# sinamalakouti/CDDMSL

Measured on AMD Instinct MI355X. Metric: images/sec (train step) VOC+Clipart RN50-C4, higher is better.
Workload: dtype bf16

## Files before the change

cddmsl_amd/csrc/roi_align.hip:

```cpp
#include "common.h"

namespace {

template <typename T> struct Vec;
template <> struct Vec<__bf16> {
  static constexpr int ES = 2, VEC = 8;
  __device__ static __forceinline__ void unpack(const u32x4& v, float* f) {
#pragma unroll
    for (int j = 0; j < 4; ++j) { f[2 * j] = bf2f(v[j] & 0xffff); f[2 * j + 1] = bf2f(v[j] >> 16); }
  }
  __device__ static __forceinline__ u32x4 pack(const float* f) {
    u32x4 v;
#pragma unroll
    for (int j = 0; j < 4; ++j) v[j] = pack2bf(f[2 * j], f[2 * j + 1]);
    return v;
  }
};
template <> struct Vec<float> {
  static constexpr int ES = 4, VEC = 4;
  __device__ static __forceinline__ void unpack(const u32x4& v, float* f) {
    const f32x4 x = __builtin_bit_cast(f32x4, v);
    f[0] = x[0]; f[1] = x[1]; f[2] = x[2]; f[3] = x[3];
  }
  __device__ static __forceinline__ u32x4 pack(const float* f) {
// ... 77 lines not shown
    const int i = i0 + rr, j = j0 + cc;
    const long bin = ((long)k * ph + i) * pw + j;
    float acc[8] = {0, 0, 0, 0, 0, 0, 0, 0};
    if (g.b >= 0 && g.b < N) {
      for (int iy = 0; iy < g.gh; ++iy) {
        int yl, yh; float wyl, wyh;
        if (tabled) {
          yl = s_lo[0][rr * g.gh + iy];
          if (yl < 0) continue;
          yh = s_hi[0][rr * g.gh + iy]; wyl = s_wl[0][rr * g.gh + iy]; wyh = s_wh[0][rr * g.gh + iy];
        } else {
          float yy = g.y0 + (float)i * g.bh + ((float)iy + 0.5f) * g.bh / (float)g.gh;
          if (!axis_tap(yy, H, yl, yh, wyl, wyh)) continue;
        }
        for (int ix = 0; ix < g.gw; ++ix) {
          int xl, xh; float wxl, wxh;
          if (tabled) {
            const int sx = j * g.gw + ix;
            xl = s_lo[1][sx];
            if (xl < 0) continue;
            xh = s_hi[1][sx]; wxl = s_wl[1][sx]; wxh = s_wh[1][sx];
          } else {
            float xx = g.x0 + (float)j * g.bw + ((float)ix + 0.5f) * g.bw / (float)g.gw;
            if (!axis_tap(xx, W, xl, xh, wxl, wxh)) continue;
          }
          float v1[8], v2[8], v3[8], v4[8];
          Vec<T>::unpack(xb[((long)yl * W + xl) * cch + c], v1);
          Vec<T>::unpack(xb[((long)yl * W + xh) * cch + c], v2);
          Vec<T>::unpack(xb[((long)yh * W + xl) * cch + c], v3);
          Vec<T>::unpack(xb[((long)yh * W + xh) * cch + c], v4);
          float w1 = wyl * wxl, w2 = wyl * wxh, w3 = wyh * wxl, w4 = wyh * wxh;
#pragma unroll
          for (int q = 0; q < VEC; ++q) {
            if (sizeof(T) == 2) {
              float tq = w1 * v1[q];
              tq = __builtin_fmaf(w2, v2[q], tq);
              tq = __builtin_fmaf(w3, v3[q], tq);
              tq = __builtin_fmaf(w4, v4[q], tq);
              acc[q] += tq;
            } else {
              acc[q] += w1 * v1[q] + w2 * v2[q] + w3 * v3[q] + w4 * v4[q];
            }
          }
        }
      }
    }
    if (pow2) {
#pragma unroll
      for (int q = 0; q < VEC; ++q) acc[q] *= inv_count;
    } else {
#pragma unroll
      for (int q = 0; q < VEC; ++q) acc[q] /= count;
    }
    if (esc) {
#pragma unroll
      for (int q = 0; q < VEC; ++q) {
        const float sq = esc[c * VEC + q], bq = ebi[c * VEC + q];
        acc[q] = sizeof(T) == 2 ? __builtin_fmaf(acc[q], sq, bq) : acc[q] * sq + bq;
        if (relu) acc[q] = fmaxf(acc[q], 0.f);
      }
    }
    outp[rr][cc] = Vec<T>::pack(acc);
    if (y) ((u32x4*)y)[bin * cch + c] = outp[rr][cc];
    if (sizeof(T) == 2 && y8) {
      float f8[8];
#pragma unroll
      for (int q = 0; q < 8; ++q) { am8 = absmax_bits(am8, acc[q]); f8[q] = __builtin_amdgcn_fmed3f(acc[q] * q8s, -448.f, 448.f); }
      int w0 = __builtin_amdgcn_cvt_pk_fp8_f32(f8[0], f8[1], 0, false), w1 = __builtin_amdgcn_cvt_pk_fp8_f32(f8[4], f8[5], 0, false);
      w0 = __builtin_amdgcn_cvt_pk_fp8_f32(f8[2], f8[3], w0, true); w1 = __builtin_amdgcn_cvt_pk_fp8_f32(f8[6], f8[7], w1, true);
      const u32x2 o8 = {(unsigned)w0, (unsigned)w1};
      ((u32x2*)y8)[bin * cch + c] = o8;
    }
    }
    if (RP == 2) {
      float a0[8], a1[8], a2[8], a3[8], o[8];
      Vec<T>::unpack(outp[0][0], a0); Vec<T>::unpack(outp[0][RP - 1], a1);
      Vec<T>::unpack(outp[RP - 1][0], a2); Vec<T>::unpack(outp[RP - 1][RP - 1], a3);
#pragma unroll
      for (int q = 0; q < VEC; ++q) o[q] = ((a0[q] + a1[q]) + (a2[q] + a3[q])) * 0.25f;
      ((u32x4*)yp)[(((long)k * (ph / 2) + i0 / 2) * (pw / 2) + j0 / 2) * cch + c] = Vec<T>::pack(o);
    }
  }
  }
  if (sizeof(T) == 2 && y8 && amax8) {
    __shared__ unsigned sm8[4];
    am8 = wave_max_u(am8);
    if ((threadIdx.x & 63) == 0) sm8[threadIdx.x >> 6] = am8;
    __syncthreads();
    if (threadIdx.x == 0) {
      unsigned m = sm8[0];
      for (int wv = 1; wv < (int)(blockDim.x >> 6); ++wv) m = sm8[wv] > m ? sm8[wv] : m;
      atomicMax(amax8 + (blockIdx.x & 63), m);
    }
  }
}

constexpr int ROW_MAXY = 32;
template <int RP>
__global__ __launch_bounds__(256) void k_roi_align_fwd_rows(const char* x, const float* rois, char* y, int N, int H, int W, int cch, int ph, int pw,
                                                            float scale, int sampling_ratio, int aligned, const float* esc, const float* ebi, int relu) {
  const int nrb = ph / RP;
  const int i0 = (blockIdx.x % nrb) * RP, k = blockIdx.x / nrb;
  const RoiGeom g = roi_geom(rois + 5 * (long)k, scale, ph, pw, sampling_ratio, aligned);
  __shared__ int s_xl[ROI_MAXS], s_py[ROW_MAXY], s_n[2];
  __shared__ float s_xwl[ROI_MAXS], s_xwh[ROI_MAXS], s_wy[ROW_MAXY];
  __shared__ int s_ylo[ROW_MAXY], s_yhi[ROW_MAXY];
  __shared__ float s_ywl[ROW_MAXY], s_ywh[ROW_MAXY];
  const int ny = RP * g.gh, nx = pw * g.gw;
  const int opw = pw / RP;
  const int c = threadIdx.x;
  const bool inb = g.b >= 0 && g.b < N;
  if (nx > ROI_MAXS || 2 * ny > ROW_MAXY || g.bw < 0.f) {
    if (c >= cch) return;
    const u32x4* xb = (const u32x4*)x + (long)(inb ? g.b : 0) * H * W * cch + c;
    const float inv = 1.0f / ((float)max(g.gh * g.gw, 1) * (float)(RP * RP));
    for (int jo = 0; jo < opw; ++jo) {
      float acc[8] = {0, 0, 0, 0, 0, 0, 0, 0};
      for (int rr = 0; rr < RP && inb; ++rr)
        for (int cc = 0; cc < RP; ++cc)
          for (int iy = 0; iy < g.gh; ++iy) {
            int yl, yh; float wyl, wyh;
            const float yy = g.y0 + (float)(i0 + rr) * g.bh + ((float)iy + 0.5f) * g.bh / (float)g.gh;
            if (!axis_tap(yy, H, yl, yh, wyl, wyh)) continue;
            for (int ix = 0; ix < g.gw; ++ix) {
              int xl, xh; float wxl, wxh;
              const float xx = g.x0 + (float)(jo * RP + cc) * g.bw + ((float)ix + 0.5f) * g.bw / (float)g.gw;
              if (!axis_tap(xx, W, xl, xh, wxl, wxh)) continue;
              float v1[8], v2[8], v3[8], v4[8];
              Vec<__bf16>::unpack(xb[((long)yl * W + xl) * cch], v1); Vec<__bf16>::unpack(xb[((long)yl * W + xh) * cch], v2);
              Vec<__bf16>::unpack(xb[((long)yh * W + xl) * cch], v3); Vec<__bf16>::unpack(xb[((long)yh * W + xh) * cch], v4);
#pragma unroll
              for (int q = 0; q < 8; ++q) acc[q] += wyl * (wxl * v1[q] + wxh * v2[q]) + wyh * (wxl * v3[q] + wxh * v4[q]);
            }
          }
      float o[8];
#pragma unroll
      for (int q = 0; q < 8; ++q) {
        o[q] = acc[q] * inv;
        if (esc) { o[q] = __builtin_fmaf(o[q], esc[c * 8 + q], ebi[c * 8 + q]); if (relu) o[q] = fmaxf(o[q], 0.f); }
      }
      ((u32x4*)y)[(((long)k * nrb + i0 / RP) * opw + jo) * cch + c] = Vec<__bf16>::pack(o);
    }
    return;
  }
  for (int s = threadIdx.x; s < ny + nx; s += blockDim.x) {
    int lo = -1, hi = -1; float wl = 0.f, wh = 0.f;
    if (s < ny) {
      const int rr = s / g.gh, iy = s - rr * g.gh;
      const float yy = g.y0 + (float)(i0 + rr) * g.bh + ((float)iy + 0.5f) * g.bh / (float)g.gh;
      if (!axis_tap(yy, H, lo, hi, wl, wh)) lo = -1;
      s_ylo[s] = lo; s_yhi[s] = hi; s_ywl[s] = wl; s_ywh[s] = wh;
    } else {
      const int sx = s - ny, j = sx / g.gw, ix = sx - j * g.gw;
      const float xx = g.x0 + (float)j * g.bw + ((float)ix + 0.5f) * g.bw / (float)g.gw;
      if (!axis_tap(xx, W, lo, hi, wl, wh)) lo = -1;
      s_xl[sx] = lo; s_xwl[sx] = wl; s_xwh[sx] = wh;
    }
  }
  __syncthreads();
  if (threadIdx.x == 0) {
    int n = 0;
    for (int s = 0; s < ny; ++s) {
      if (s_ylo[s] < 0) continue;
      const int r2[2] = {s_ylo[s], s_yhi[s]};
      const float w2[2] = {s_ywl[s], s_ywh[s]};
      for (int e = 0; e < 2; ++e) {
        int f = -1;
        for (int q = 0; q < n; ++q) if (s_py[q] == r2[e]) f = q;
        if (f < 0) { f = n++; s_py[f] = r2[e]; s_wy[f] = 0.f; }
        s_wy[f] += w2[e];
      }
    }
    int first = -1;
    for (int s = 0; s < nx && first < 0; ++s) if (s_xl[s] >= 0) first = s_xl[s];
    s_n[0] = n; s_n[1] = first;
  }
  __syncthreads();
  const int lane = threadIdx.x & 63;
  int xlr[ROI_MAXS / 64], xwlr[ROI_MAXS / 64], xwhr[ROI_MAXS / 64];
#pragma unroll
  for (int q = 0; q < ROI_MAXS / 64; ++q) {
    const int idx = q * 64 + lane;
    const bool in = idx < nx;
    xlr[q] = in ? s_xl[idx] : -1;
    xwlr[q] = in ? __builtin_bit_cast(int, s_xwl[idx]) : 0;
    xwhr[q] = in ? __builtin_bit_cast(int, s_xwh[idx]) : 0;
  }
  if (c >= cch) return;
  const int nrow = __builtin_amdgcn_readfirstlane(s_n[0]);
  const int first = __builtin_amdgcn_readfirstlane(s_n[1]);
  const float inv = 1.0f / ((float)max(g.gh * g.gw, 1) * (float)(RP * RP));
  float sq[8], bq[8];
#pragma unroll
  for (int q = 0; q < 8; ++q) { sq[q] = esc ? esc[c * 8 + q] : 1.f; bq[q] = ebi ? ebi[c * 8 + q] : 0.f; }
  const u32x4* xb = (const u32x4*)x + (long)(inb ? g.b : 0) * H * W * cch + c;
  auto rload = [&](int px, float* R) {
#pragma unroll
    for (int q = 0; q < 8; ++q) R[q] = 0.f;
    for (int e = 0; e < nrow; ++e) {
      const int py = __builtin_amdgcn_readfirstlane(s_py[e]);
      const float wy = __builtin_bit_cast(float, __builtin_amdgcn_readfirstlane(__builtin_bit_cast(int, s_wy[e])));
      float v[8];
      Vec<__bf16>::unpack(xb[((long)py * W + px) * cch], v);
#pragma unroll
      for (int q = 0; q < 8; ++q) R[q] = __builtin_fmaf(wy, v[q], R[q]);
    }
  };
  float R0[8], R1[8], acc[8];
#pragma unroll
  for (int q = 0; q < 8; ++q) { R0[q] = R1[q] = acc[q] = 0.f; }
  int cur = first;
  const bool any = inb && nrow > 0 && first >= 0;
  constexpr int PF = 4;
  const bool ahead = nrow <= PF;
  int pyr[PF]; float wyr[PF];
#pragma unroll
  for (int e = 0; e < PF; ++e) {
    pyr[e] = __builtin_amdgcn_readfirstlane(s_py[e < nrow ? e : 0]);
    wyr[e] = e < nrow ? __builtin_bit_cast(float, __builtin_amdgcn_readfirstlane(__builtin_bit_cast(int, s_wy[e]))) : 0.f;
  }
  u32x4 raw[PF];
  auto issue = [&](int px) {
#pragma unroll
    for (int e = 0; e < PF; ++e) if (e < nrow) raw[e] = xb[((long)pyr[e] * W + px) * cch];
  };
  auto finish = [&](float* R) {
#pragma unroll
    for (int q = 0; q < 8; ++q) R[q] = 0.f;
#pragma unroll
    for (int e = 0; e < PF; ++e) if (e < nrow) {
      float v[8];
      Vec<__bf16>::unpack(raw[e], v);
#pragma unroll
      for (int q = 0; q < 8; ++q) R[q] = __builtin_fmaf(wyr[e], v[q], R[q]);
    }
  };
  if (any) {
    rload(cur, R0); rload(min(cur + 1, W - 1), R1);
    if (ahead) issue(min(cur + 2, W - 1));
  }
  const int spo = RP * g.gw;
  u32x4* yo = (u32x4*)y + ((long)k * nrb + i0 / RP) * opw * cch + c;
  if (nx == 0) {
    float o[8];
#pragma unroll
    for (int q = 0; q < 8; ++q) { o[q] = 0.f; if (esc) { o[q] = bq[q]; if (relu) o[q] = fmaxf(o[q], 0.f); } }
    for (int jo = 0; jo < opw; ++jo) yo[(long)jo * cch] = Vec<__bf16>::pack(o);
    return;
  }
  int left = spo, j = 0;
#pragma unroll
  for (int q = 0; q < ROI_MAXS / 64; ++q) {
  const int lim = min(64, nx - q * 64);
  for (int l = 0; l < lim; ++l) {
    const int xl = __builtin_amdgcn_readlane(xlr[q], l);
    if (any && xl >= 0) {
      while (cur < xl) {
        ++cur;
#pragma unroll
        for (int q = 0; q < 8; ++q) R0[q] = R1[q];
        if (ahead) { finish(R1); issue(min(cur + 2, W - 1)); }
        else rload(min(cur + 1, W - 1), R1);
      }
      const float wl = __builtin_bit_cast(float, __builtin_amdgcn_readlane(xwlr[q], l));
      const float wh = __builtin_bit_cast(float, __builtin_amdgcn_readlane(xwhr[q], l));
#pragma unroll
      for (int q = 0; q < 8; ++q) acc[q] = __builtin_fmaf(wl, R0[q], __builtin_fmaf(wh, R1[q], acc[q]));
    }
    if (--left == 0) {
      float o[8];
#pragma unroll
      for (int q = 0; q < 8; ++q) {
        o[q] = acc[q] * inv;
        if (esc) { o[q] = __builtin_fmaf(o[q], sq[q], bq[q]); if (relu) o[q] = fmaxf(o[q], 0.f); }
        acc[q] = 0.f;
      }
      __builtin_nontemporal_store(Vec<__bf16>::pack(o), &yo[(long)j * cch]);
      ++j; left = spo;
    }
  }
  }
}

__global__ void k_roi_tables(const float* rois, float* ay, float* ax, int* fp, int K, int H, int W, int ph, int pw,
                             float scale, int sampling_ratio, int aligned, int fold) {
  int k = blockIdx.x;
  RoiGeom g = roi_geom(rois + 5 * (long)k, scale, ph * fold, pw * fold, sampling_ratio, aligned);
  float* ayk = ay + (long)k * H * ph;
  float* axk = ax + (long)k * W * pw;
  for (int i = threadIdx.x; i < H * ph; i += blockDim.x) ayk[i] = 0.f;
  for (int i = threadIdx.x; i < W * pw; i += blockDim.x) axk[i] = 0.f;
  __shared__ int lim[4];
  if (threadIdx.x == 0) { lim[0] = H; lim[1] = -1; lim[2] = W; lim[3] = -1; }
  __syncthreads();
  const float fw = 1.0f / (float)fold;
  if (threadIdx.x < ph) {
    int lo_min = H, hi_max = -1;
    for (int i = threadIdx.x * fold; i < (threadIdx.x + 1) * fold; ++i)
    for (int iy = 0; iy < g.gh; ++iy) {
      float yy = g.y0 + (float)i * g.bh + ((float)iy + 0.5f) * g.bh / (float)g.gh;
      int yl, yh; float wl, wh;
      if (!axis_tap(yy, H, yl, yh, wl, wh)) continue;
      ayk[yl * ph + threadIdx.x] += fw * (wl / (float)g.gh);
      ayk[yh * ph + threadIdx.x] += fw * (wh / (float)g.gh);
      lo_min = min(lo_min, yl); hi_max = max(hi_max, yh);
    }
    atomicMin(&lim[0], lo_min); atomicMax(&lim[1], hi_max);
  } else if (threadIdx.x >= 64 && threadIdx.x < 64 + pw) {
    const int jc = threadIdx.x - 64;
    int lo_min = W, hi_max = -1;
    for (int j = jc * fold; j < (jc + 1) * fold; ++j)
    for (int ix = 0; ix < g.gw; ++ix) {
      float xx = g.x0 + (float)j * g.bw + ((float)ix + 0.5f) * g.bw / (float)g.gw;
      int xl, xh; float wl, wh;
      if (!axis_tap(xx, W, xl, xh, wl, wh)) continue;
      axk[xl * pw + jc] += fw * (wl / (float)g.gw);
      axk[xh * pw + jc] += fw * (wh / (float)g.gw);
      lo_min = min(lo_min, xl); hi_max = max(hi_max, xh);
    }
    atomicMin(&lim[2], lo_min); atomicMax(&lim[3], hi_max);
  }
  __syncthreads();
  if (threadIdx.x == 0) {
    bool ok = g.b >= 0;
    fp[4 * k] = ok ? lim[0] : 1; fp[4 * k + 1] = ok ? lim[1] : 0; fp[4 * k + 2] = lim[2]; fp[4 * k + 3] = lim[3];
  }
}

// ... 47 lines not shown
      for (int a = 0; a < TS; ++a) wyi[a] = __builtin_bit_cast(float, __builtin_amdgcn_readlane(__builtin_bit_cast(int, wyv[a]), i));
      unsigned long long xm = xm0;
      while (xm) {
        const int j = __builtin_ctzll(xm);
        xm &= xm - 1;
        float wxj[TS];
#pragma unroll
        for (int a = 0; a < TS; ++a) wxj[a] = __builtin_bit_cast(float, __builtin_amdgcn_readlane(__builtin_bit_cast(int, wxv[a]), j));
        const u32x4* src = (const u32x4*)dy + (((long)k * ph + i) * pw + j) * cch;
        float v[NC][8];
#pragma unroll
        for (int u = 0; u < NC; ++u) {
          const int c = threadIdx.x + u * blockDim.x;
          if (c < cch) Vec<T>::unpack(src[c], v[u]);
        }
#pragma unroll
        for (int a = 0; a < TS; ++a)
#pragma unroll
          for (int b = 0; b < TS; ++b) {
            const float w = wyi[a] * wxj[b];
            if (w == 0.f) continue;
#pragma unroll
            for (int u = 0; u < NC; ++u)
#pragma unroll
              for (int q = 0; q < VEC; ++q) acc[u][a * TS + b][q] += w * v[u][q];
          }
      }
    }
  }
  }
#pragma unroll
  for (int u = 0; u < NC; ++u) {
    const int c = threadIdx.x + u * blockDim.x;
    if (c < cch) {
#pragma unroll
      for (int a = 0; a < TS; ++a)
#pragma unroll
        for (int b = 0; b < TS; ++b)
          if (py0 + a < H && px0 + b < W) ((u32x4*)dx)[(((long)n * H + py0 + a) * W + px0 + b) * cch + c] = Vec<T>::pack(acc[u][a * TS + b]);
    }
  }
}

}

static int roi_align_forward_impl(const void* x, const float* rois, void* y, void* y_pooled, int* dbg_grid, const float* esc,
                                  const float* ebi, int relu, int N, int C, int H, int W, int K, int ph, int pw, float spatial_scale,
                                  int sampling_ratio, int aligned, int dtype, void* stream, void* y8 = nullptr, const float* q8 = nullptr,
                                  float* amax8 = nullptr) {
  int es = dtype == 0 ? 2 : 4;
  if ((dtype != 0 && dtype != 1) || (C * es) % 16 || H <= 0 || W <= 0 || ph <= 0 || pw <= 0 || K < 0 || N < 0)
    return CDDMSL_ERR_ARG;
  if ((esc == nullptr) != (ebi == nullptr)) return CDDMSL_ERR_ARG;
  if (K == 0) return CDDMSL_OK;
  if (!y && !y_pooled) return CDDMSL_ERR_ARG;
  if (y8 && (dtype != 0 || !y)) return CDDMSL_ERR_ARG;
  int cch = C * es / 16;
  if (y_pooled && ((ph & 1) || (pw & 1))) return CDDMSL_ERR_ARG;
  long grid = (long)K * (y_pooled ? ph / 2 : ph);
  if (grid > 0x7fffffffL) return CDDMSL_ERR_ARG;
  int threads = cch >= 256 ? 256 : ((cch + 63) / 64) * 64;
  hipStream_t st = (hipStream_t)stream;
  const char* rows_env = getenv("CDDMSL_ROI_ROWS");
  const bool rows_off = rows_env && rows_env[0] == '0';
  if (dtype == 0 && !y8 && !dbg_grid && ((y != nullptr) != (y_pooled != nullptr)) && cch <= 256 && !rows_off) {
    if (y) k_roi_align_fwd_rows<1><<<dim3((unsigned)((long)K * ph)), dim3(threads), 0, st>>>((const char*)x, rois, (char*)y, N, H, W, cch, ph, pw, spatial_scale, sampling_ratio, aligned, esc, ebi, relu);
    else k_roi_align_fwd_rows<2><<<dim3((unsigned)((long)K * (ph / 2))), dim3(threads), 0, st>>>((const char*)x, rois, (char*)y_pooled, N, H, W, cch, ph, pw, spatial_scale, sampling_ratio, aligned, esc, ebi, relu);
    return launch_status();
  }
#define CDDMSL_RAF(TT, RPP) k_roi_align_fwd<TT, RPP><<<dim3((unsigned)grid), dim3(threads), 0, st>>>((const char*)x, rois, (char*)y, (char*)y_pooled, dbg_grid, N, H, W, cch, ph, pw, spatial_scale, sampling_ratio, aligned, esc, ebi, relu, (char*)y8, q8, (unsigned*)amax8)
  if (dtype == 0) { if (y_pooled) CDDMSL_RAF(__bf16, 2); else CDDMSL_RAF(__bf16, 1); }
  else { if (y_pooled) CDDMSL_RAF(float, 2); else CDDMSL_RAF(float, 1); }
#undef CDDMSL_RAF
  return launch_status();
}

extern "C" int cddmsl_roi_align_forward(const void* x, const float* rois, void* y, void* y_pooled, int* dbg_grid, int N, int C,
                                        int H, int W, int K, int ph, int pw, float spatial_scale, int sampling_ratio,
                                        int aligned, int dtype, void* stream) {
  if (!y && K > 0) return CDDMSL_ERR_ARG;
  return roi_align_forward_impl(x, rois, y, y_pooled, dbg_grid, nullptr, nullptr, 0, N, C, H, W, K, ph, pw, spatial_scale,
                                sampling_ratio, aligned, dtype, stream);
}

extern "C" int cddmsl_roi_align_forward_affine(const void* x, const float* rois, void* y, void* y_pooled, const float* scale,
                                               const float* bias, int relu, int N, int C, int H, int W, int K, int ph, int pw,
                                               float spatial_scale, int sampling_ratio, int aligned, int dtype, void* y8,
                                               const float* q8, float* amax8, void* stream) {
  return roi_align_forward_impl(x, rois, y, y_pooled, nullptr, scale, bias, relu, N, C, H, W, K, ph, pw, spatial_scale,
                                sampling_ratio, aligned, dtype, stream, y8, q8, amax8);
}

static int roi_align_backward_impl(const void* dy, const float* rois, const int* roi_start, void* dx, float* ws_ay,
                                   float* ws_ax, int* ws_fp, int N, int C, int H, int W, int K, int ph, int pw,
                                   float spatial_scale, int sampling_ratio, int aligned, int dtype, int fold, void* stream) {
  int es = dtype == 0 ? 2 : 4;
  if ((dtype != 0 && dtype != 1) || (C * es) % 16 || H <= 0 || W <= 0 || ph <= 0 || pw <= 0 || K < 0 || N < 0)
    return CDDMSL_ERR_ARG;
  if (ph > MAXP || pw > MAXP || ph > 64 || pw > 64) return CDDMSL_ERR_ARG;
  int cch = C * es / 16;
  if (cch > 1024) return CDDMSL_ERR_ARG;
  hipStream_t st = (hipStream_t)stream;
  if (N == 0) return CDDMSL_OK;
  if (K > 0) k_roi_tables<<<dim3((unsigned)K), dim3(128), 0, st>>>(rois, ws_ay, ws_ax, ws_fp, K, H, W, ph, pw, spatial_scale, sampling_ratio, aligned, fold);
  int threads = cch >= 256 ? 256 : ((cch + 63) / 64) * 64;
  const int ncpt = (cch + threads - 1) / threads;
  const int ts = 2;
  long grid = (long)N * ((H + ts - 1) / ts) * ((W + ts - 1) / ts);
  if (grid > 0x7fffffffL) return CDDMSL_ERR_ARG;
#define CDDMSL_RAB(TT, NCC, TSS) k_roi_align_bwd<TT, NCC, TSS><<<dim3((unsigned)grid), dim3(threads), 0, st>>>((const char*)dy, ws_ay, ws_ax, ws_fp, roi_start, (char*)dx, H, W, cch, ph, pw)
  if (dtype == 0) { if (ncpt <= 1) CDDMSL_RAB(__bf16, 1, 2); else if (ncpt == 2) CDDMSL_RAB(__bf16, 2, 2); else CDDMSL_RAB(__bf16, 4, 2); }
  else { if (ncpt <= 1) CDDMSL_RAB(float, 1, 2); else if (ncpt == 2) CDDMSL_RAB(float, 2, 2); else CDDMSL_RAB(float, 4, 2); }
#undef CDDMSL_RAB
  return launch_status();
}

extern "C" int cddmsl_roi_align_backward(const void* dy, const float* rois, const int* roi_start, void* dx, float* ws_ay,
                                         float* ws_ax, int* ws_fp, int N, int C, int H, int W, int K, int ph, int pw,
                                         float spatial_scale, int sampling_ratio, int aligned, int dtype, void* stream) {
  return roi_align_backward_impl(dy, rois, roi_start, dx, ws_ay, ws_ax, ws_fp, N, C, H, W, K, ph, pw, spatial_scale,
// ... 112 lines not shown
```

cddmsl_amd/hip.py:

```python
import ctypes
import os
from ctypes import c_float, c_int, c_long, c_void_p

import torch

from ._lib import check, lib, ptr, require_cuda, stream_ptr

DT = {torch.bfloat16: 0, torch.float32: 1}

_sigs_done = False


def _L():
    global _sigs_done
    L = lib()
    if not _sigs_done:
        vp, ci, cf = c_void_p, c_int, c_float
        L.cddmsl_last_kernel.argtypes = []
        L.cddmsl_plan_only.argtypes = [ci]
        L.cddmsl_conv_fwd.argtypes = [vp] * 7 + [ci] * 16 + [vp]
        L.cddmsl_bottleneck64_ok.argtypes = [ci] * 4
        L.cddmsl_bottleneck64_fwd.argtypes = [vp] * 17 + [ci] * 4 + [vp]
        L.cddmsl_conv_wgrad.argtypes = [vp] * 4 + [ci] * 12 + [vp]
        L.cddmsl_set_workspace.argtypes = [vp, c_long]
# ... 649 lines not shown
    return dx


@_timed("colsum")
def colsum(x2d, period=1, out=None):
    require_cuda(x2d, out)
    rows, cols = x2d.shape
    assert x2d.is_contiguous()
    if out is None:
        out = torch.zeros((period, cols) if period > 1 else (cols,), device=x2d.device, dtype=torch.float32)
    check(_L().cddmsl_colsum(ptr(x2d), ptr(out), rows, cols, period, _dt(x2d), stream_ptr()), "cddmsl_colsum")
    return out


def same_layout(a, b):
    return a.shape == b.shape and all(sa == sb for sa, sb, n in zip(a.stride(), b.stride(), a.shape) if n > 1)


@_timed("sgd_clip_step")
def sgd_clip_step(params, grads, moms, norm_ws, lr, momentum, wd, clip, first_step):
    n = len(params)
    if n == 0:
        return
    require_cuda(*params, *grads, *moms)
    for p, g, m in zip(params, grads, moms):
        assert p.dtype == g.dtype == m.dtype == torch.float32
        assert same_layout(p, g) and same_layout(p, m), "param/grad/momentum must share a memory layout"
    P = (c_void_p * n)(*[p.data_ptr() for p in params])
    G = (c_void_p * n)(*[g.data_ptr() for g in grads])
    M = (c_void_p * n)(*[m.data_ptr() for m in moms])
    S = (c_long * n)(*[p.numel() for p in params])
    check(_L().cddmsl_sgd_clip_step(P, G, M, S, n, ptr(norm_ws), lr, momentum, wd, clip, int(first_step), stream_ptr()),
          "cddmsl_sgd_clip_step")


@_timed("roi_align_forward")
def roi_align_forward(x, rois, ph, pw, spatial_scale, sampling_ratio, aligned, dbg_grid=None, with_pooled=False, extra_rows=0):
    require_cuda(x, rois)
    assert rois.dim() == 2 and rois.size(1) == 5 and rois.dtype == torch.float32 and rois.is_contiguous()
    N, H, W, C = x.shape
    K = rois.shape[0]
    y = torch.empty((K + extra_rows, ph, pw, C), device=x.device, dtype=x.dtype)
    yp = torch.empty((K + extra_rows, ph // 2, pw // 2, C), device=x.device, dtype=x.dtype) if with_pooled else None
    check(_L().cddmsl_roi_align_forward(ptr(x), ptr(rois), ptr(y), ptr(yp), ptr(dbg_grid), N, C, H, W, K, ph, pw, spatial_scale,
                                         sampling_ratio, int(aligned), _dt(x), stream_ptr()), "cddmsl_roi_align_forward")
    return (y, yp) if with_pooled else y


@_timed("roi_align_forward")
def roi_align_forward_affine(x, rois, ph, pw, spatial_scale, sampling_ratio, aligned, scale=None, bias=None, relu=False,
                             pooled_only=False, extra_rows=0, emit8=None):
    require_cuda(x, rois)
    assert rois.dim() == 2 and rois.size(1) == 5 and rois.dtype == torch.float32 and rois.is_contiguous()
    assert (scale is None) == (bias is None) and not (pooled_only and scale is not None)
    N, H, W, C = x.shape
    K = rois.shape[0]
    if pooled_only:
        y, yp = None, torch.empty((K + extra_rows, ph // 2, pw // 2, C), device=x.device, dtype=x.dtype)
    else:
        y, yp = torch.empty((K + extra_rows, ph, pw, C), device=x.device, dtype=x.dtype), None
        assert scale is None or (scale.dtype == torch.float32 and scale.numel() == C and bias.numel() == C and scale.is_contiguous() and bias.is_contiguous())
    y8 = None
    if emit8 is not None:
        assert not pooled_only and x.dtype == torch.bfloat16
        y8 = torch.empty(y.shape, device=x.device, dtype=torch.uint8)
    check(_L().cddmsl_roi_align_forward_affine(ptr(x), ptr(rois), ptr(y), ptr(yp), ptr(scale), ptr(bias), int(relu), N, C, H, W, K,
                                                ph, pw, spatial_scale, sampling_ratio, int(aligned), _dt(x), ptr(y8),
                                                ptr(emit8[0]) if emit8 else c_void_p(0), ptr(emit8[1]) if emit8 else c_void_p(0), stream_ptr()),
          "cddmsl_roi_align_forward_affine")
    if y8 is not None:
        y._fp8 = (y8, emit8[0].data_ptr())
    return yp if pooled_only else y


@_timed("roi_align_backward")
def roi_align_backward(dy, rois, roi_start, in_shape, spatial_scale, sampling_ratio, aligned, pooled=False):
    require_cuda(dy, rois, roi_start)
    N, H, W, C = in_shape
    K, ph, pw, _ = dy.shape
    assert roi_start.dtype == torch.int32 and roi_start.numel() == N + 1 and dy.is_contiguous()
    dx = torch.empty(in_shape, device=dy.device, dtype=dy.dtype)
    ay = workspace("roi_ay", max(K, 1) * H * ph * 4, dy.device)
    ax = workspace("roi_ax", max(K, 1) * W * pw * 4, dy.device)
    fp = workspace("roi_fp", max(K, 1) * 16, dy.device)
    fn = _L().cddmsl_roi_align_backward_pooled if pooled else _L().cddmsl_roi_align_backward
    check(fn(ptr(dy), ptr(rois), ptr(roi_start), ptr(dx), ptr(ay), ptr(ax), ptr(fp), N, C, H, W, K,
             ph, pw, spatial_scale, sampling_ratio, int(aligned), _dt(dy), stream_ptr()), "cddmsl_roi_align_backward")
    return dx


def roi_align_nchw(input, rois, output_size, spatial_scale, sampling_ratio, aligned):
    require_cuda(input, rois)
    assert rois.dim() == 2 and rois.size(1) == 5 and rois.dtype == torch.float32 and rois.is_contiguous() and input.is_contiguous()
    N, C, H, W = input.shape
    ph, pw = (output_size, output_size) if isinstance(output_size, int) else output_size
    K = rois.shape[0]
    out = torch.zeros((K, C, ph, pw), device=input.device, dtype=input.dtype)
    nbytes = ctypes.c_size_t(0)
    args = (N, C, H, W, K, ph, pw, spatial_scale, sampling_ratio, int(aligned), _dt(input))
    check(_L().cddmsl_roi_align_nchw_anyorder(ptr(input), ptr(rois), ptr(out), *args, None, ctypes.byref(nbytes), stream_ptr()), "cddmsl_roi_align_nchw_anyorder(size)")
    ws = workspace("roi_nchw", max(nbytes.value, 1), input.device)
    check(_L().cddmsl_roi_align_nchw_anyorder(ptr(input), ptr(rois), ptr(out), *args, ptr(ws), ctypes.byref(nbytes), stream_ptr()), "cddmsl_roi_align_nchw_anyorder")
    return out


def roi_align_backward_nchw(grad, rois, input_shape, spatial_scale, sampling_ratio, aligned):
    require_cuda(grad, rois)
    assert rois.dtype == torch.float32 and rois.is_contiguous() and grad.is_contiguous()
    N, C, H, W = input_shape
    K, _, ph, pw = grad.shape
    dx = torch.zeros(tuple(input_shape), device=grad.device, dtype=grad.dtype)
    nbytes = ctypes.c_size_t(0)
    args = (N, C, H, W, K, ph, pw, spatial_scale, sampling_ratio, int(aligned), _dt(grad))
    check(_L().cddmsl_roi_align_backward_nchw_anyorder(ptr(grad), ptr(rois), ptr(dx), *args, None, ctypes.byref(nbytes), stream_ptr()), "cddmsl_roi_align_backward_nchw_anyorder(size)")
# ... 586 lines not shown
```

cddmsl_amd/layers.py:

```python
import os
import weakref

import torch

from . import hip

_STEP = [0]


def bump_weight_version():
    _STEP[0] += 1


_LOAD_GEN = [0]


def note_weights_loaded(*_):
    _LOAD_GEN[0] += 1
    _STEP[0] += 1


def load_generation():
    return _LOAD_GEN[0]

# ... 550 lines not shown


def _fused_stage_forward(x, blocks):
    T = x.dtype
    wf = lambda pw: pw.get(T, need_dgrad=False)[0]
    o1 = conv_fwd_auto(x, blocks[0].pw[0], blocks[0].bn[0][0], blocks[0].bn[0][1], False, relu=True)
    cur = x
    for bi, bp in enumerate(blocks):
        nxt = blocks[bi + 1] if bi + 1 < len(blocks) else None
        kw = dict(x0=cur, wd=wf(bp.pw[3]), bnd=bp.bn[3]) if bp.pw[3] is not None else dict(residual=cur)
        if nxt is not None:
            kw.update(w1n=wf(nxt.pw[0]), bn1n=nxt.bn[0])
        cur, o1 = hip.bottleneck64_fwd(o1, wf(bp.pw[1]), bp.bn[1], wf(bp.pw[2]), bp.bn[2], **kw)
    return cur


def res_stage(x, blocks, frozen, out_grad_premasked=False, out_spec=None):
    px0 = getattr(x, "_pooled2", None)
    if frozen or not torch.is_grad_enabled():
        if _fused_stage_ok(x, blocks, out_spec):
            return _fused_stage_forward(x, blocks)
        cur = x
        for bi, bp in enumerate(blocks):
            cur, _ = _block_forward(cur, bp, False, px0 if bi == 0 else None, blocks[bi + 1].pw[0] if bi + 1 < len(blocks) else None,
                                    out_spec if bi + 1 == len(blocks) else None)
        return cur
    return ResStageFn.apply(x, blocks[0].w[0], blocks, out_grad_premasked, px0, out_spec)


class StackHalvesFn(torch.autograd.Function):

    @staticmethod
    def forward(ctx, a, b, full):
        n = a.shape[0]
        assert a.data_ptr() == full.data_ptr() and b.data_ptr() == full[n:].data_ptr() and full.shape[0] == 2 * n and a.shape == b.shape
        ctx.n = n
        return full.view(full.shape)

    @staticmethod
    def backward(ctx, g):
        return g[:ctx.n], g[ctx.n:], None


def stack_halves(a, b, full):
    return StackHalvesFn.apply(a, b, full)


def res_stage_attnpool(x, blocks, frozen, ap):
    fuse = not frozen and torch.is_grad_enabled()
    y = res_stage(x, blocks, frozen, out_grad_premasked=fuse)
    return AttnPoolFn.apply(y, None if ap.frozen else ap.q_w, ap, fuse)


def _roi_block0_forward(feat, rois, bp, out_size, scale, sr, extra, next_pw=None):
    T = feat.dtype
    (s1, b1), (s2, b2), (s3, b3), bnd = bp.bn
    w1, _ = bp.pw[0].get(T, False)
    f8 = bp.fp8
    K, E = rois.shape[0], (0 if extra is None else extra.shape[0])
    z = hip.conv_fwd(feat, w1)
    o1_shape = (K + E, out_size, out_size, z.shape[-1])
    e8 = fp8_emit_for(bp.pw[1], o1_shape, 1, f8) if E == 0 else None
    o1 = hip.roi_align_forward_affine(z, rois, out_size, out_size, scale, sr, True, s1, b1, relu=True, extra_rows=E, emit8=e8)
    px = hip.roi_align_forward_affine(feat, rois, out_size, out_size, scale, sr, True, pooled_only=True, extra_rows=E)
    if E:
        o1[K:].copy_(hip.conv_fwd(extra, w1, s1, b1, relu=True))
        px[K:].copy_(hip.avgpool2_fwd(extra))
    o2 = conv_fwd_auto(o1, bp.pw[1], s2, b2, f8, relu=True, pad=1)
    p2 = hip.avgpool2_fwd(o2)
    idn = conv_fwd_auto(px, bp.pw[3], bnd[0], bnd[1], f8)
    out_shape = (p2.shape[0], p2.shape[1], p2.shape[2], _ohwi(bp.w[2]).shape[0])
    out = conv_fwd_auto(p2, bp.pw[2], s3, b3, f8, emit8=fp8_emit_for(next_pw, out_shape, 0, f8), residual=idn, relu=True)
    return o1, o2, p2, px, out, (_fp8_made_for(o1, bp.pw[1]) if f8 else None)


class RoIStageFn(torch.autograd.Function):

    @staticmethod
    def forward(ctx, feat, anchor, rois, roi_start, blocks, out_size, scale, sr, out_grad_premasked, extra):
        feat = feat.contiguous()
        nxt = lambda i: blocks[i + 1].pw[0] if i + 1 < len(blocks) else None
        o1, o2, p2, px, cur, o1_8 = _roi_block0_forward(feat, rois, blocks[0], out_size, scale, sr, extra, nxt(0))
        saved, o1_8s = [feat, rois, roi_start, extra, o1, o2, p2, px, cur], [None, o1_8, None]
        for bi, bp in enumerate(blocks[1:], start=1):
            cur, mids = _block_forward(cur, bp, True, None, nxt(bi))
            saved += [mids[0], mids[1], mids[2], mids[3], cur]
            o1_8s += list(mids[4])
        ctx.blocks, ctx.meta = blocks, (out_size, scale, sr, out_grad_premasked)
        ctx.save_for_backward(*saved, *o1_8s)
        return cur

    @staticmethod
    def backward(ctx, g):
        blocks = ctx.blocks
        saved, o1_8s = ctx.saved_tensors[:-3 * len(blocks)], ctx.saved_tensors[-3 * len(blocks):]
        out_size, scale, sr, premasked = ctx.meta
        feat, rois, roi_start, extra = saved[:4]
        st = saved[4:]
        gs = g.contiguous() if premasked else hip.relu_bwd(g.contiguous(), st[-1])
        for i in range(len(blocks) - 1, 0, -1):
            o1, o2, p2, px = st[5 * i: 5 * i + 4]
            gs = _block_backward(gs, st[5 * i - 1], o1, o2, p2, px, blocks[i], True, mask_x=True, prev_bp=blocks[i - 1], c8=tuple(o1_8s[3 * i: 3 * i + 3]))
        bp = blocks[0]
        o1, o2, p2, px = st[0:4]
        T = o1.dtype
        (s1, _), (s2, _), (s3, _), bnd = bp.bn
        w1p, w2p, w3p, wdp = bp.w
        shp = lambda w: _ohwi(w).shape
        K, E = rois.shape[0], (0 if extra is None else extra.shape[0])
        f8 = bp.fp8 and T == torch.bfloat16
        gs_slot = fp8_slot_of(bp, "_fp8_gs") if f8 else None
        d2_slot = fp8_slot_of(bp.pw[1], "_fp8_g") if f8 else None
        hip.conv_wgrad(p2, gs, shp(w3p), s3, out=_ohwi(_grad_buf(w3p)))
        e8 = d2_slot.emit() if f8 and _fp8_dgrad_wanted(bp.pw[1], o2.shape, 1, f8) else None
        dpre2 = hip.avgpool2_bwd(dgrad_auto(gs, bp.pw[2], f8, gs_slot), tuple(o2.shape), mask=o2, emit8=e8)
        dpre1 = dgrad_auto(dpre2, bp.pw[1], f8, d2_slot, pad=1, relu_mask=o1)
        wgrad_auto(o1, dpre2, bp.pw[1], s2, 1, _ohwi(_grad_buf(w2p)), f8, o1_8s[1], d2_slot)
        hip.conv_wgrad(px, gs, shp(wdp), bnd[0], out=_ohwi(_grad_buf(wdp)))
        dxb = dgrad_auto(gs, bp.pw[3], f8, gs_slot)
        N, H, W, C = feat.shape
        dz = hip.roi_align_backward(dpre1[:K], rois, roi_start, (N, H, W, dpre1.shape[-1]), scale, sr, True)
        hip.conv_wgrad(feat, dz, shp(w1p), s1, out=_ohwi(_grad_buf(w1p)))
        _, w1d = bp.pw[0].get(T, True)
        dfeat = dextra = None
        if E:
            hip.conv_wgrad(extra, dpre1[K:], shp(w1p), s1, out=_ohwi(_grad_buf(w1p)))
            if ctx.needs_input_grad[9]:
                dextra = hip.conv_fwd(dpre1[K:], w1d, residual=hip.avgpool2_bwd(dxb[K:].contiguous(), tuple(extra.shape)))
        if ctx.needs_input_grad[0]:
            r = hip.roi_align_backward(dxb[:K], rois, roi_start, (N, H, W, C), scale, sr, True, pooled=True)
            dfeat = hip.conv_fwd(dz, w1d, residual=r)
        return dfeat, None, None, None, None, None, None, None, None, dextra


def roi_stage_supported(blocks):
    bp = blocks[0]
    return bp.stride == 2 and bp.w[3] is not None and tuple(bp.w[0].shape[2:]) == (1, 1) and tuple(bp.w[3].shape[2:]) == (1, 1)


def roi_stage(feat, rois, roi_start, blocks, frozen, out_size, scale, sr, extra=None, out_grad_premasked=False):
    assert rois.dim() == 2 and rois.size(1) == 5 and out_size % 2 == 0
    assert extra is None or tuple(extra.shape[1:]) == (out_size, out_size, feat.shape[3])
    if frozen or not torch.is_grad_enabled():
        nxt = lambda i: blocks[i + 1].pw[0] if i + 1 < len(blocks) else None
        cur = _roi_block0_forward(feat.contiguous(), rois, blocks[0], out_size, scale, sr, extra, nxt(0))[4]
        for bi, bp in enumerate(blocks[1:], start=1):
            cur, _ = _block_forward(cur, bp, False, None, nxt(bi))
        return cur
    return RoIStageFn.apply(feat, blocks[0].w[0], rois, roi_start, blocks, out_size, scale, sr, out_grad_premasked, extra)


def roi_stage_attnpool(feat, rois, roi_start, blocks, frozen, ap, out_size, scale, sr, extra=None):
    fuse = not frozen and torch.is_grad_enabled()
    y = roi_stage(feat, rois, roi_start, blocks, frozen, out_size, scale, sr, extra, out_grad_premasked=fuse)
    return AttnPoolFn.apply(y, None if ap.frozen else ap.q_w, ap, fuse)


class RoIAlignFn(torch.autograd.Function):
    @staticmethod
    def forward(ctx, x, rois, roi_start, out_size, scale, sampling_ratio, aligned, with_pooled=False, extra=None):
        K, E = rois.shape[0], (0 if extra is None else extra.shape[0])
        out = hip.roi_align_forward(x, rois, out_size, out_size, scale, sampling_ratio, aligned, with_pooled=with_pooled, extra_rows=E)
        ctx.save_for_backward(rois, roi_start)
        ctx.meta = (tuple(x.shape), scale, sampling_ratio, aligned, K)
        y = out[0] if with_pooled else out
        if E:
            y[K:].copy_(extra)
            if with_pooled:
                out[1][K:].copy_(hip.avgpool2_fwd(extra.contiguous()))
        if with_pooled:
            ctx.mark_non_differentiable(out[1])
        return out

    @staticmethod
    def backward(ctx, dy, *unused):
        rois, roi_start = ctx.saved_tensors
        shape, scale, sr, aligned, K = ctx.meta
        dy = dy.contiguous()
        dx = hip.roi_align_backward(dy[:K], rois, roi_start, shape, scale, sr, aligned)
        dextra = dy[K:] if (dy.shape[0] > K and ctx.needs_input_grad[8]) else None
        return dx, None, None, None, None, None, None, None, dextra


# ... 397 lines not shown
```

Before: 158.5.

## Commute downsample 1x1 conv before RoIAlign when RoI outputs exceed map size

Because RoIAlign is linear, the downsample branch's 1x1 conv is now applied to the full feature map and then pooled (with the BN affine folded into the pooled RoIAlign), instead of RoIAligning the input and convolving per RoI. This applies when K*(out/2)^2 exceeds N*H*W, and backward is rewritten to match: RoIAlign-backward the gradient first, then run wgrad/dgrad on the map. The rows kernel also moves to a 2D grid with 64-thread blocks over channels and hoists the affine loads. This trades per-RoI conv work for map-sized conv work, and bf16 rounding order changes slightly.

```diff
diff --git a/cddmsl_amd/csrc/roi_align.hip b/cddmsl_amd/csrc/roi_align.hip
--- a/cddmsl_amd/csrc/roi_align.hip
+++ b/cddmsl_amd/csrc/roi_align.hip
@@ -153,7 +153,7 @@
 #pragma unroll
       for (int q = 0; q < VEC; ++q) acc[q] /= count;
     }
-    if (esc) {
+    if (esc && !(RP == 2 && !y)) {
 #pragma unroll
       for (int q = 0; q < VEC; ++q) {
         const float sq = esc[c * VEC + q], bq = ebi[c * VEC + q];
@@ -179,6 +179,13 @@
       Vec<T>::unpack(outp[RP - 1][0], a2); Vec<T>::unpack(outp[RP - 1][RP - 1], a3);
 #pragma unroll
       for (int q = 0; q < VEC; ++q) o[q] = ((a0[q] + a1[q]) + (a2[q] + a3[q])) * 0.25f;
+      if (esc && !y) {
+#pragma unroll
+        for (int q = 0; q < VEC; ++q) {
+          const float sq = esc[c * VEC + q], bq = ebi[c * VEC + q];
+          o[q] = sizeof(T) == 2 ? __builtin_fmaf(o[q], sq, bq) : o[q] * sq + bq;
+        }
+      }
       ((u32x4*)yp)[(((long)k * (ph / 2) + i0 / 2) * (pw / 2) + j0 / 2) * cch + c] = Vec<T>::pack(o);
     }
   }
@@ -209,8 +216,16 @@
   __shared__ float s_ywl[ROW_MAXY], s_ywh[ROW_MAXY];
   const int ny = RP * g.gh, nx = pw * g.gw;
   const int opw = pw / RP;
-  const int c = threadIdx.x;
+  const int c = blockIdx.y * blockDim.x + threadIdx.x;
   const bool inb = g.b >= 0 && g.b < N;
+  float sq[8], bq[8];
+#pragma unroll
+  for (int q = 0; q < 8; ++q) { sq[q] = 1.f; bq[q] = 0.f; }
+  if (esc) {
+    const int cl = min(c, cch - 1);
+#pragma unroll
+    for (int q = 0; q < 8; ++q) { sq[q] = esc[cl * 8 + q]; bq[q] = ebi[cl * 8 + q]; }
+  }
   if (nx > ROI_MAXS || 2 * ny > ROW_MAXY || g.bw < 0.f) {
     if (c >= cch) return;
     const u32x4* xb = (const u32x4*)x + (long)(inb ? g.b : 0) * H * W * cch + c;
@@ -238,7 +253,7 @@
 #pragma unroll
       for (int q = 0; q < 8; ++q) {
         o[q] = acc[q] * inv;
-        if (esc) { o[q] = __builtin_fmaf(o[q], esc[c * 8 + q], ebi[c * 8 + q]); if (relu) o[q] = fmaxf(o[q], 0.f); }
+        if (esc) { o[q] = __builtin_fmaf(o[q], sq[q], bq[q]); if (relu) o[q] = fmaxf(o[q], 0.f); }
       }
       ((u32x4*)y)[(((long)k * nrb + i0 / RP) * opw + jo) * cch + c] = Vec<__bf16>::pack(o);
     }
@@ -291,9 +306,6 @@
   const int nrow = __builtin_amdgcn_readfirstlane(s_n[0]);
   const int first = __builtin_amdgcn_readfirstlane(s_n[1]);
   const float inv = 1.0f / ((float)max(g.gh * g.gw, 1) * (float)(RP * RP));
-  float sq[8], bq[8];
-#pragma unroll
-  for (int q = 0; q < 8; ++q) { sq[q] = esc ? esc[c * 8 + q] : 1.f; bq[q] = ebi ? ebi[c * 8 + q] : 0.f; }
   const u32x4* xb = (const u32x4*)x + (long)(inb ? g.b : 0) * H * W * cch + c;
   auto rload = [&](int px, float* R) {
 #pragma unroll
@@ -336,6 +348,7 @@
       for (int q = 0; q < 8; ++q) R[q] = __builtin_fmaf(wyr[e], v[q], R[q]);
     }
   };
+  __builtin_amdgcn_s_waitcnt(0x0F70);
   if (any) {
     rload(cur, R0); rload(min(cur + 1, W - 1), R1);
     if (ahead) issue(min(cur + 2, W - 1));
@@ -371,10 +384,14 @@
     if (--left == 0) {
       float o[8];
 #pragma unroll
-      for (int q = 0; q < 8; ++q) {
-        o[q] = acc[q] * inv;
-        if (esc) { o[q] = __builtin_fmaf(o[q], sq[q], bq[q]); if (relu) o[q] = fmaxf(o[q], 0.f); }
-        acc[q] = 0.f;
+      for (int q = 0; q < 8; ++q) { o[q] = acc[q] * inv; acc[q] = 0.f; }
+      if (esc) {
+#pragma unroll
+        for (int q = 0; q < 8; ++q) o[q] = __builtin_fmaf(o[q], sq[q], bq[q]);
+        if (relu) {
+#pragma unroll
+          for (int q = 0; q < 8; ++q) o[q] = fmaxf(o[q], 0.f);
+        }
       }
       __builtin_nontemporal_store(Vec<__bf16>::pack(o), &yo[(long)j * cch]);
       ++j; left = spo;
@@ -528,6 +545,7 @@
   if ((dtype != 0 && dtype != 1) || (C * es) % 16 || H <= 0 || W <= 0 || ph <= 0 || pw <= 0 || K < 0 || N < 0)
     return CDDMSL_ERR_ARG;
   if ((esc == nullptr) != (ebi == nullptr)) return CDDMSL_ERR_ARG;
+  if (!y && y_pooled && relu) return CDDMSL_ERR_ARG;
   if (K == 0) return CDDMSL_OK;
   if (!y && !y_pooled) return CDDMSL_ERR_ARG;
   if (y8 && (dtype != 0 || !y)) return CDDMSL_ERR_ARG;
@@ -540,8 +558,10 @@
   const char* rows_env = getenv("CDDMSL_ROI_ROWS");
   const bool rows_off = rows_env && rows_env[0] == '0';
   if (dtype == 0 && !y8 && !dbg_grid && ((y != nullptr) != (y_pooled != nullptr)) && cch <= 256 && !rows_off) {
-    if (y) k_roi_align_fwd_rows<1><<<dim3((unsigned)((long)K * ph)), dim3(threads), 0, st>>>((const char*)x, rois, (char*)y, N, H, W, cch, ph, pw, spatial_scale, sampling_ratio, aligned, esc, ebi, relu);
-    else k_roi_align_fwd_rows<2><<<dim3((unsigned)((long)K * (ph / 2))), dim3(threads), 0, st>>>((const char*)x, rois, (char*)y_pooled, N, H, W, cch, ph, pw, spatial_scale, sampling_ratio, aligned, esc, ebi, relu);
+    const int rthreads = 64;
+    const unsigned gy = (unsigned)((cch + rthreads - 1) / rthreads);
+    if (y) k_roi_align_fwd_rows<1><<<dim3((unsigned)((long)K * ph), gy), dim3(rthreads), 0, st>>>((const char*)x, rois, (char*)y, N, H, W, cch, ph, pw, spatial_scale, sampling_ratio, aligned, esc, ebi, relu);
+    else k_roi_align_fwd_rows<2><<<dim3((unsigned)((long)K * (ph / 2)), gy), dim3(rthreads), 0, st>>>((const char*)x, rois, (char*)y_pooled, N, H, W, cch, ph, pw, spatial_scale, sampling_ratio, aligned, esc, ebi, relu);
     return launch_status();
   }
 #define CDDMSL_RAF(TT, RPP) k_roi_align_fwd<TT, RPP><<<dim3((unsigned)grid), dim3(threads), 0, st>>>((const char*)x, rois, (char*)y, (char*)y_pooled, dbg_grid, N, H, W, cch, ph, pw, spatial_scale, sampling_ratio, aligned, esc, ebi, relu, (char*)y8, q8, (unsigned*)amax8)
diff --git a/cddmsl_amd/hip.py b/cddmsl_amd/hip.py
--- a/cddmsl_amd/hip.py
+++ b/cddmsl_amd/hip.py
@@ -725,14 +725,14 @@
                              pooled_only=False, extra_rows=0, emit8=None):
     require_cuda(x, rois)
     assert rois.dim() == 2 and rois.size(1) == 5 and rois.dtype == torch.float32 and rois.is_contiguous()
-    assert (scale is None) == (bias is None) and not (pooled_only and scale is not None)
+    assert (scale is None) == (bias is None)
     N, H, W, C = x.shape
     K = rois.shape[0]
     if pooled_only:
         y, yp = None, torch.empty((K + extra_rows, ph // 2, pw // 2, C), device=x.device, dtype=x.dtype)
     else:
         y, yp = torch.empty((K + extra_rows, ph, pw, C), device=x.device, dtype=x.dtype), None
-        assert scale is None or (scale.dtype == torch.float32 and scale.numel() == C and bias.numel() == C and scale.is_contiguous() and bias.is_contiguous())
+    assert scale is None or (scale.dtype == torch.float32 and scale.numel() == C and bias.numel() == C and scale.is_contiguous() and bias.is_contiguous())
     y8 = None
     if emit8 is not None:
         assert not pooled_only and x.dtype == torch.bfloat16
diff --git a/cddmsl_amd/layers.py b/cddmsl_amd/layers.py
--- a/cddmsl_amd/layers.py
+++ b/cddmsl_amd/layers.py
@@ -626,23 +626,49 @@
     return AttnPoolFn.apply(y, None if ap.frozen else ap.q_w, ap, fuse)
 
 
-def _roi_block0_forward(feat, rois, bp, out_size, scale, sr, extra, next_pw=None):
+def roi_downsample_on_map(K, out_size, N, H, W):
+    if os.environ.get("CDDMSL_ROI_COMMUTE", "1") == "0":
+        return False
+    v = os.environ.get("CDDMSL_ROI_COMMUTE_DOWN", "")
+    if v in ("0", "1"):
+        return v == "1"
+    return K * (out_size // 2) ** 2 > N * H * W
+
+
+def _roi_block0_forward(feat, rois, bp, out_size, scale, sr, extra, next_pw=None, on_map=None):
     T = feat.dtype
     (s1, b1), (s2, b2), (s3, b3), bnd = bp.bn
     w1, _ = bp.pw[0].get(T, False)
     f8 = bp.fp8
     K, E = rois.shape[0], (0 if extra is None else extra.shape[0])
+    N, H, W, _ = feat.shape
     z = hip.conv_fwd(feat, w1)
     o1_shape = (K + E, out_size, out_size, z.shape[-1])
     e8 = fp8_emit_for(bp.pw[1], o1_shape, 1, f8) if E == 0 else None
     o1 = hip.roi_align_forward_affine(z, rois, out_size, out_size, scale, sr, True, s1, b1, relu=True, extra_rows=E, emit8=e8)
-    px = hip.roi_align_forward_affine(feat, rois, out_size, out_size, scale, sr, True, pooled_only=True, extra_rows=E)
+    del z
+    if on_map is None:
+        on_map = roi_downsample_on_map(K, out_size, N, H, W)
+    if on_map:
+        wd, _ = bp.pw[3].get(T, False)
+        zd = hip.conv_fwd(feat, wd)
+        idn = hip.roi_align_forward_affine(zd, rois, out_size, out_size, scale, sr, True, bnd[0], bnd[1], pooled_only=True, extra_rows=E)
+        del zd
+        px = None
+        if E:
+            px = hip.avgpool2_fwd(extra)
+            idn[K:].copy_(hip.conv_fwd(px, wd, bnd[0], bnd[1]))
+    else:
+        px = hip.roi_align_forward_affine(feat, rois, out_size, out_size, scale, sr, True, pooled_only=True, extra_rows=E)
+        idn = None
     if E:
         o1[K:].copy_(hip.conv_fwd(extra, w1, s1, b1, relu=True))
-        px[K:].copy_(hip.avgpool2_fwd(extra))
+        if idn is None:
+            px[K:].copy_(hip.avgpool2_fwd(extra))
     o2 = conv_fwd_auto(o1, bp.pw[1], s2, b2, f8, relu=True, pad=1)
     p2 = hip.avgpool2_fwd(o2)
-    idn = conv_fwd_auto(px, bp.pw[3], bnd[0], bnd[1], f8)
+    if idn is None:
+        idn = conv_fwd_auto(px, bp.pw[3], bnd[0], bnd[1], f8)
     out_shape = (p2.shape[0], p2.shape[1], p2.shape[2], _ohwi(bp.w[2]).shape[0])
     out = conv_fwd_auto(p2, bp.pw[2], s3, b3, f8, emit8=fp8_emit_for(next_pw, out_shape, 0, f8), residual=idn, relu=True)
     return o1, o2, p2, px, out, (_fp8_made_for(o1, bp.pw[1]) if f8 else None)
@@ -654,13 +680,14 @@
     def forward(ctx, feat, anchor, rois, roi_start, blocks, out_size, scale, sr, out_grad_premasked, extra):
         feat = feat.contiguous()
         nxt = lambda i: blocks[i + 1].pw[0] if i + 1 < len(blocks) else None
-        o1, o2, p2, px, cur, o1_8 = _roi_block0_forward(feat, rois, blocks[0], out_size, scale, sr, extra, nxt(0))
+        on_map = roi_downsample_on_map(rois.shape[0], out_size, feat.shape[0], feat.shape[1], feat.shape[2])
+        o1, o2, p2, px, cur, o1_8 = _roi_block0_forward(feat, rois, blocks[0], out_size, scale, sr, extra, nxt(0), on_map)
         saved, o1_8s = [feat, rois, roi_start, extra, o1, o2, p2, px, cur], [None, o1_8, None]
         for bi, bp in enumerate(blocks[1:], start=1):
             cur, mids = _block_forward(cur, bp, True, None, nxt(bi))
             saved += [mids[0], mids[1], mids[2], mids[3], cur]
             o1_8s += list(mids[4])
-        ctx.blocks, ctx.meta = blocks, (out_size, scale, sr, out_grad_premasked)
+        ctx.blocks, ctx.meta = blocks, (out_size, scale, sr, out_grad_premasked, on_map)
         ctx.save_for_backward(*saved, *o1_8s)
         return cur
 
@@ -668,7 +695,7 @@
     def backward(ctx, g):
         blocks = ctx.blocks
         saved, o1_8s = ctx.saved_tensors[:-3 * len(blocks)], ctx.saved_tensors[-3 * len(blocks):]
-        out_size, scale, sr, premasked = ctx.meta
+        out_size, scale, sr, premasked, on_map = ctx.meta
         feat, rois, roi_start, extra = saved[:4]
         st = saved[4:]
         gs = g.contiguous() if premasked else hip.relu_bwd(g.contiguous(), st[-1])
@@ -690,19 +717,27 @@
         dpre2 = hip.avgpool2_bwd(dgrad_auto(gs, bp.pw[2], f8, gs_slot), tuple(o2.shape), mask=o2, emit8=e8)
         dpre1 = dgrad_auto(dpre2, bp.pw[1], f8, d2_slot, pad=1, relu_mask=o1)
         wgrad_auto(o1, dpre2, bp.pw[1], s2, 1, _ohwi(_grad_buf(w2p)), f8, o1_8s[1], d2_slot)
-        hip.conv_wgrad(px, gs, shp(wdp), bnd[0], out=_ohwi(_grad_buf(wdp)))
-        dxb = dgrad_auto(gs, bp.pw[3], f8, gs_slot)
         N, H, W, C = feat.shape
+        _, w1d = bp.pw[0].get(T, True)
+        dfeat = dextra = dzd = wdd = None
+        if on_map:
+            _, wdd = bp.pw[3].get(T, True)
+            dzd = hip.roi_align_backward(gs[:K], rois, roi_start, (N, H, W, gs.shape[-1]), scale, sr, True, pooled=True)
+            hip.conv_wgrad(feat, dzd, shp(wdp), bnd[0], out=_ohwi(_grad_buf(wdp)))
+            if E:
+                hip.conv_wgrad(px, gs[K:], shp(wdp), bnd[0], out=_ohwi(_grad_buf(wdp)))
+        else:
+            hip.conv_wgrad(px, gs, shp(wdp), bnd[0], out=_ohwi(_grad_buf(wdp)))
+            dxb = dgrad_auto(gs, bp.pw[3], f8, gs_slot)
         dz = hip.roi_align_backward(dpre1[:K], rois, roi_start, (N, H, W, dpre1.shape[-1]), scale, sr, True)
         hip.conv_wgrad(feat, dz, shp(w1p), s1, out=_ohwi(_grad_buf(w1p)))
-        _, w1d = bp.pw[0].get(T, True)
-        dfeat = dextra = None
         if E:
             hip.conv_wgrad(extra, dpre1[K:], shp(w1p), s1, out=_ohwi(_grad_buf(w1p)))
             if ctx.needs_input_grad[9]:
-                dextra = hip.conv_fwd(dpre1[K:], w1d, residual=hip.avgpool2_bwd(dxb[K:].contiguous(), tuple(extra.shape)))
+                dxe = hip.conv_fwd(gs[K:], wdd) if on_map else dxb[K:].contiguous()
+                dextra = hip.conv_fwd(dpre1[K:], w1d, residual=hip.avgpool2_bwd(dxe, tuple(extra.shape)))
         if ctx.needs_input_grad[0]:
-            r = hip.roi_align_backward(dxb[:K], rois, roi_start, (N, H, W, C), scale, sr, True, pooled=True)
+            r = hip.conv_fwd(dzd, wdd) if on_map else hip.roi_align_backward(dxb[:K], rois, roi_start, (N, H, W, C), scale, sr, True, pooled=True)
             dfeat = hip.conv_fwd(dz, w1d, residual=r)
         return dfeat, None, None, None, None, None, None, None, None, dextra
 
```

Measured after the change: 162.8, median of 6. 2.7% higher.
